# centreborelli/sat-bundleadjust

Measured on NVIDIA B200. Metric: lm_observation_iterations_per_s, higher is better.
Workload: dtype f64

## Files before the change

sat_bundleadjust_b200/csrc/sba_internal.cuh:

```cuda
#pragma once
#include <cuda_runtime.h>
#include <stdint.h>
#include <stdio.h>
#include <string>
#include <vector>

#include "../../include/sba_b200.h"
#include "sba_models.cuh"

namespace sba {

void set_error(const std::string& msg);

#define SBA_CUDA(expr)                                                                              \
    do {                                                                                            \
        cudaError_t _e = (expr);                                                                    \
        if (_e != cudaSuccess) {                                                                    \
            ::sba::set_error(std::string(#expr) + ": " + cudaGetErrorString(_e) + " (" + __FILE__ + ":" + \
                             std::to_string(__LINE__) + ")");                                       \
            return SBA_E_CUDA;                                                                      \
        }                                                                                           \
    } while (0)

#define SBA_TRY(expr)                \
// ... 73 lines not shown
    int *slice_block = nullptr, *slice_p0 = nullptr, *slice_p1 = nullptr;
    long long n_pairs = 0;
    int *tile_obs = nullptr;
    int n_tiles = 0;
    int n_schur_blocks = 0;

    double *x = nullptr, *x_new = nullptr, *g = nullptr, *sinv = nullptr, *delta = nullptr, *t1 = nullptr, *t2 = nullptr;
    double *camrec = nullptr, *camrec_new = nullptr;
    double *V = nullptr, *F = nullptr, *q = nullptr, *Z = nullptr;
    double *camsys_local = nullptr, *camsys = nullptr;
    double *S = nullptr;
    bool comm_split = false;
    int n_common = 0;
    double *cvec = nullptr;
    double *chol_work = nullptr;
    double *cam_partials = nullptr, *schur_partials = nullptr, *red_partials = nullptr;
    unsigned* counters = nullptr;
    double* scal = nullptr;
    double* h_scal = nullptr;
    double* r_out = nullptr;
    double* err_out = nullptr;
    double *io_x = nullptr;
    cudaEvent_t ev0 = nullptr, ev1 = nullptr;
    int launches = 0;
    std::vector<cudaEvent_t> ev_pool;
    int ev_used = 0;
    void* comm_buf = nullptr;
    void* comm_peer[16] = {nullptr};
    long long comm_cap = 0;
    unsigned long long comm_seq = 0;
    bool comm_ready = false;
    std::vector<void*> arena_chunks;
    std::vector<size_t> arena_chunk_bytes;
    char* arena_ptr = nullptr;
    size_t arena_left = 0;
    void* flush_buf = nullptr;
    size_t flush_bytes = 0;

    bool use_pcg = false;
    double pcg_tol = 1e-8;
    int pcg_max_it = 500;
    long long pcg_iterations = 0, pcg_solves = 0;
    double *pcg_vec = nullptr, *pcg_diag = nullptr, *pcg_L = nullptr, *pcg_w = nullptr, *pcg_s = nullptr;

    int engine = 0;
    int n_pts_fix_int = 0;
    std::vector<int> h_trk_new2old, h_obs_new2old;
    int *trk_new2old = nullptr, *obs_new2old = nullptr;
    void* pt_units[3] = {nullptr, nullptr, nullptr};
    int* pt_warp_unit0[3] = {nullptr, nullptr, nullptr};
    int pt_n_cta = 0;
    double *V2 = nullptr, *g2 = nullptr, *camsys2 = nullptr;
    long long* pt_cycles = nullptr;
    bool pt_obs_uploaded = false;
    bool pt_schur_mma = false;
    double *dsq = nullptr, *idsq = nullptr;
    double *dsqc = nullptr, *dsqc2 = nullptr, *idsqc = nullptr, *idsqc2 = nullptr;
    double *pt_partials = nullptr;
    double *osc = nullptr, *osc2 = nullptr;
    double *pt_records = nullptr;
    double *r_int = nullptr, *e_int = nullptr;
};
```

sat_bundleadjust_b200/csrc/sba_pattern.cuh:

```cuda
#pragma once
#include "sba_comm.cuh"
#include "sba_kernels.cuh"
#include "sba_pattern.h"

namespace sba {

constexpr int PT_CTAS = NUM_SMS;
constexpr int PT_THREADS = 512;
constexpr int PT_THREADS_LIGHT = 512;
constexpr int PT_THREADS_SCHUR = 384;
constexpr int PT_MAX_NS = 132;
constexpr int PT_RC = 3;

struct PatView {
    const PUnit* units;
    const int* warp_unit0;
    const double2* pts2d;
    const double* w;
    const double* cam_static;
    const double* rpc_tab;
    int M, P, n_cam_fix, n_cta;
    int debug_skip;
    long long* cycles;
};

__device__ __forceinline__ double step_value2(double x, double t, double d, double pa, double pb)
{
    return x + fma(pa, t, pb * d);
}

__device__ __forceinline__ bool invert_point_block_d2(double v0, double v1, double v2, double v3, double v4, double v5,
                                                      double d0, double d1, double d2, double reg, double G[6])
{
    const double a00 = v0 + reg * d0, a10 = v1, a20 = v2;
    const double a11 = v3 + reg * d1, a21 = v4, a22 = v5 + reg * d2;
    bool ok = a00 > 0.0;
    const double i00 = fast_rsqrt(a00);
    const double c10 = a10 * i00, c20 = a20 * i00;
    const double d11 = a11 - c10 * c10;
    ok = ok && d11 > 0.0;
    const double i11 = fast_rsqrt(d11);
    const double c21 = (a21 - c20 * c10) * i11;
    const double d22 = a22 - c20 * c20 - c21 * c21;
    ok = ok && d22 > 0.0;
    const double i22 = fast_rsqrt(d22);
    if (!ok) {
#pragma unroll
        for (int k = 0; k < 6; ++k) G[k] = 0.0;
        return false;
    }
    G[0] = i00; G[2] = i11; G[5] = i22;
    G[1] = -c10 * i00 * i11;
    G[4] = -c21 * i11 * i22;
    G[3] = -(c20 * i00 + c21 * G[1]) * i22;
    return true;
}

template <int NV>
__device__ __forceinline__ double cta_reduce_sum(double (&v)[NV], double* sm)
{
    warp_reduce_sum<NV>(v);
    const int lane = threadIdx.x & 31, warp = threadIdx.x >> 5, nw = blockDim.x >> 5;
    __syncthreads();
    if (lane == 0) {
#pragma unroll
        for (int k = 0; k < NV; ++k) sm[warp * NV + k] = v[k];
    }
    __syncthreads();
    double s = 0.0;
    if (threadIdx.x < NV)
        for (int wq = 0; wq < nw; ++wq) s += sm[wq * NV + threadIdx.x];
    __syncthreads();
    return s;
}

template <int NV>
__device__ __forceinline__ bool grid_sum_last(double block_total, double* partials, unsigned* counter, double* scal,
// ... 22 lines not shown
__device__ __forceinline__ void load_cameras_shared(const PatView& A, const double* __restrict__ camrec, double* s_cam,
                                                    double* s_rpc)
{
    for (int t = threadIdx.x; t < A.M * CAMREC_STRIDE; t += blockDim.x) s_cam[t] = camrec[t];
    if (MODEL == MODEL_RPC)
        for (int t = threadIdx.x; t < A.M * RPC_TAB_STRIDE; t += blockDim.x) s_rpc[t] = A.rpc_tab[t];
}

__device__ __forceinline__ int unit_camera(const PUnit& u, int k)
{
    const int nlo = __popc(u.mask_lo);
    return k < nlo ? (int)__fns(u.mask_lo, 0, k + 1) : 32 + (int)__fns(u.mask_hi, 0, k - nlo + 1);
}

struct LaneGeo {
    int L, T, k, t, cam;
    bool on;
};
__device__ __forceinline__ LaneGeo lane_geometry(const PUnit& u, int lane)
{
    LaneGeo g;
    g.L = u.L; g.T = min(32 / u.L, PT_MAX_T);
    g.t = lane / u.L; g.k = lane - g.t * u.L;
    g.on = g.t < g.T;
    g.cam = g.on ? unit_camera(u, g.k) : 0;
    return g;
}

__device__ __forceinline__ double slot_reduce(double v, const LaneGeo& g)
{
    for (int off = 1; off < g.T; off <<= 1) {
        const double o = __shfl_down_sync(0xffffffffu, v, (unsigned)(off * g.L) & 31);
        if (g.on && g.t + off < g.T) v += o;
    }
    return v;
}

template <int N>
__device__ __forceinline__ void slot_reduce_n(double (&v)[N], const LaneGeo& g)
{
    for (int off = 1; off < g.T; off <<= 1) {
        const unsigned delta = (unsigned)(off * g.L) & 31;
        const bool take = g.on && g.t + off < g.T;
        double o[N];
#pragma unroll
        for (int q = 0; q < N; ++q) o[q] = __shfl_down_sync(0xffffffffu, v[q], delta);
#pragma unroll
        for (int q = 0; q < N; ++q) if (take) v[q] += o[q];
    }
}

__device__ __forceinline__ void prefetch_l1(const void* p) { asm volatile("prefetch.global.L1 [%0];" ::"l"(p)); }

template <int MODEL, int NC>
__device__ __forceinline__ void eval_scaled(const double* __restrict__ rec, const double* __restrict__ rpc_j, double X, double Y,
                                            double Z, double2 sc, bool cam_free, bool pt_free, ObsEval<MODEL, NC>& e)
{
    double u, v;
    full_side<MODEL, NC, true>(rec, rpc_j, X, Y, Z, u, v, e.Jc, e.Jp);
    const double a0 = cam_free ? sc.x : 0.0, a1 = cam_free ? sc.y : 0.0;
#pragma unroll
    for (int k = 0; k < NC; ++k) { e.Jc[k] *= a0; e.Jc[NC + k] *= a1; }
    const double b0 = pt_free ? sc.x : 0.0, b1 = pt_free ? sc.y : 0.0;
#pragma unroll
    for (int k = 0; k < 3; ++k) { e.Jp[k] *= b0; e.Jp[3 + k] *= b1; }
}

template <int MODEL, int NC>
__global__ void __launch_bounds__(PT_THREADS, 1)
k_pt_assemble(PatView A, const double* __restrict__ x, const double* __restrict__ g, const double* __restrict__ idsq,
              const double* __restrict__ idsq_c, const double* __restrict__ delta, const double* __restrict__ scal,
              int initial, int ns, int loss, double f_scale, double* __restrict__ x_new, double* __restrict__ camrec_new,
              double* __restrict__ V_new, double* __restrict__ g_new, double2* __restrict__ osc_new, double* __restrict__ partials)
{
    constexpr int NU = NC * (NC + 1) / 2, NV = NU + NC;
    extern __shared__ double smem[];
    double* s_cam = smem;
    double* s_rpc = s_cam + A.M * CAMREC_STRIDE;
    double* s_acc = s_rpc + (MODEL == MODEL_RPC ? A.M * RPC_TAB_STRIDE : 0);
    const int lane = threadIdx.x & 31, warp = threadIdx.x >> 5, nw = blockDim.x >> 5;
    double* s_stage = s_acc + nw * A.M * NV;
    double* s_red = s_stage + nw * 9 * 33;
    const double pa = initial ? 0.0 : scal[SC_PA], pb = initial ? 0.0 : scal[SC_PB];
    if (threadIdx.x < A.M) {
        const int j = threadIdx.x;
        double v[MAX_CAM_PARAMS];
#pragma unroll
        for (int s = 0; s < MAX_CAM_PARAMS; ++s) {
            double val = 0.0;
            if (s < A.P) {
                if (s < NC) {
                    const size_t e = (size_t)j * NC + s;
                    const double xv = initial ? x[e] : step_value2(x[e], g[e] * idsq_c[e], delta[e], pa, pb);
                    if (blockIdx.x == 0) x_new[e] = xv;
                    val = j >= A.n_cam_fix ? xv : A.cam_static[(size_t)j * A.P + s];
                } else {
                    val = A.cam_static[(size_t)j * A.P + s];
                }
            }
            v[s] = val;
        }
        build_camrec(v, MODEL, s_cam + j * CAMREC_STRIDE);
    }
    if (MODEL == MODEL_RPC)
        for (int t = threadIdx.x; t < A.M * RPC_TAB_STRIDE; t += blockDim.x) s_rpc[t] = A.rpc_tab[t];
    for (int t = threadIdx.x; t < nw * A.M * NV; t += blockDim.x) s_acc[t] = 0.0;
    __syncthreads();
    if (blockIdx.x == 0)
        for (int t = threadIdx.x; t < A.M * CAMREC_STRIDE; t += blockDim.x) camrec_new[t] = s_cam[t];

    double cost[1] = {0.0};
    double* stg = s_stage + warp * 9 * 33;
    double* my_acc = s_acc + warp * A.M * NV;
    const int u0 = A.warp_unit0[blockIdx.x * nw + warp], u1 = A.debug_skip ? u0 : A.warp_unit0[blockIdx.x * nw + warp + 1];
    const long long cyc0 = clock64();
    for (int u = u0; u < u1; ++u) {
        const PUnit un = A.units[u];
        const LaneGeo G = lane_geometry(un, lane);
        const bool cam_free = G.cam >= A.n_cam_fix, pt_free = un.pts_free != 0;
        const double* rec = s_cam + G.cam * CAMREC_STRIDE;
        const double* rpc_j = MODEL == MODEL_RPC ? s_rpc + G.cam * RPC_TAB_STRIDE : nullptr;
        double acc[NV];
#pragma unroll
        for (int q = 0; q < NV; ++q) acc[q] = 0.0;
        for (int tb = 0; tb < un.ntrk; tb += G.T) {
            const int tt = tb + G.t;
            const bool on = G.on && tt < un.ntrk;
            const int nact = min(G.T, un.ntrk - tb);
// ... 58 lines not shown
            __syncwarp();
            for (int s = lane; s < 9 * nact; s += 32) {
                const int tr = s / 9, q = s - 9 * tr;
                const double* src = stg + q * 33 + tr * G.L;
                double tsum = 0.0;
                for (int m = 0; m < G.L; ++m) tsum += src[m];
                const int it = un.trk0 + tb + tr;
                if (q < 6) V_new[6 * (size_t)it + q] = tsum;
                else g_new[(size_t)ns + 3 * (size_t)it + (q - 6)] = tsum;
            }
            __syncwarp();
        }
        slot_reduce_n<NV>(acc, G);
        if (G.on && G.t == 0) {
            double* dst = my_acc + G.cam * NV;
#pragma unroll
            for (int q = 0; q < NV; ++q) dst[q] += acc[q];
        }
        __syncwarp();
    }
    if (A.cycles && lane == 0) A.cycles[blockIdx.x * nw + warp] = clock64() - cyc0;
    const double ctot = cta_reduce_sum<1>(cost, s_red);
    for (int t = threadIdx.x; t < A.M * NV; t += blockDim.x) {
        double sum = 0.0;
        for (int wq = 0; wq < nw; ++wq) sum += s_acc[wq * A.M * NV + t];
        partials[(size_t)t * A.n_cta + blockIdx.x] = sum;
    }
    if (threadIdx.x == 0) partials[(size_t)A.M * NV * A.n_cta + blockIdx.x] = ctot;
}

__device__ __forceinline__ void cam_scale_dev(const double* __restrict__ camsys, const double* __restrict__ dsq_c_cur,
                                              int first, int M, int NC, double* __restrict__ dsq_c_new,
                                              double* __restrict__ idsq_c_new, double* __restrict__ g_new, double* scal)
{
    const int ns = M * NC;
    for (int e = threadIdx.x; e < ns; e += blockDim.x) {
        const int j = e / NC, s = e - j * NC;
        const double diag = __ldcg(camsys + (size_t)j * NC * NC + s * NC + s);
        const double d = first ? (diag == 0.0 ? 1.0 : diag) : fmax(dsq_c_cur[e], diag);
        dsq_c_new[e] = d;
        idsq_c_new[e] = 1.0 / d;
        g_new[e] = __ldcg(camsys + (size_t)M * NC * NC + e);
    }
    if (threadIdx.x == 0) scal[SC_COST_NEW] = __ldcg(camsys + (size_t)M * NC * NC + ns);
}

template <int NC>
__global__ void __launch_bounds__(256)
k_pt_reduce_assemble(const double* __restrict__ partials, int n_cta, int M, double* __restrict__ camsys, int fold,
                     const double* __restrict__ dsq_c_cur, int first, double* __restrict__ dsq_c_new,
                     double* __restrict__ idsq_c_new, double* __restrict__ g_new, double* scal, unsigned* counter, CommFused comm)
{
    constexpr int NU = NC * (NC + 1) / 2, NV = NU + NC;
    const int lane = threadIdx.x & 31;
    const int total = M * NV + 1;
    const int v = blockIdx.x * (blockDim.x >> 5) + (threadIdx.x >> 5);
    if (v < total) {
        double s = 0.0;
        for (int b = lane; b < n_cta; b += 32) s += partials[(size_t)v * n_cta + b];
#pragma unroll
        for (int o = 16; o > 0; o >>= 1) s += __shfl_xor_sync(0xffffffffu, s, o);
        if (lane == 0) {
            if (v == M * NV) {
                camsys[(size_t)M * NC * NC + (size_t)M * NC] = s;
            } else {
                const int j = v / NV, q = v - j * NV;
                if (q < NU) {
                    int r = 0;
                    while ((r + 1) * (r + 2) / 2 <= q) ++r;
                    const int c = q - r * (r + 1) / 2;
                    camsys[(size_t)j * NC * NC + r * NC + c] = s;
                    camsys[(size_t)j * NC * NC + c * NC + r] = s;
                } else {
                    camsys[(size_t)M * NC * NC + (size_t)j * NC + (q - NU)] = s;
                }
            }
        }
    }
    if (!fold) return;
    __shared__ bool is_last;
    __threadfence();
    __syncthreads();
    if (threadIdx.x == 0) is_last = (atomicAdd(counter, 1u) == gridDim.x - 1);
    __syncthreads();
    if (!is_last) return;
    __threadfence();
    if (threadIdx.x == 0) *counter = 0u;
    if (comm.on) cta_allreduce(comm.c, camsys, M * NC * NC + M * NC + 1, comm.seq, scal);
    cam_scale_dev(camsys, dsq_c_cur, first, M, NC, dsq_c_new, idsq_c_new, g_new, scal);
}

__global__ void __launch_bounds__(256)
k_pt_cam_scale(const double* __restrict__ camsys, const double* __restrict__ dsq_c_cur, int first, int M, int NC,
               double* __restrict__ dsq_c_new, double* __restrict__ idsq_c_new, double* __restrict__ g_new, double* scal)
{
    cam_scale_dev(camsys, dsq_c_cur, first, M, NC, dsq_c_new, idsq_c_new, g_new, scal);
}

__device__ __forceinline__ void control_reg_dev(double* scal, double delta_arg, double reg_override)
{
    double Delta = delta_arg;
    if (Delta < 0.0) {
        Delta = sqrt(scal[SC_XS]);
        if (Delta == 0.0) Delta = 1.0;
    }
    scal[SC_DELTA] = Delta;
    if (reg_override >= 0.0) { scal[SC_REG] = reg_override; return; }
    const double gg = scal[SC_GG];
    const double qa = 0.5 * scal[SC_A], qb = -gg;
    const double to_tr = Delta / sqrt(gg);
    double ag = 0.0;
    ag = fmin(ag, to_tr * (qa * to_tr + qb));
    if (qa != 0.0) {
        const double ext = -0.5 * qb / qa;
        if (ext > 0.0 && ext < to_tr) ag = fmin(ag, ext * (qa * ext + qb));
    }
    scal[SC_REG] = -ag / (Delta * Delta);
}

__device__ __forceinline__ void control_tr2d_gram_dev(double* scal, double delta_arg)
{
    const double Delta = delta_arg < 0.0 ? scal[SC_DELTA] : delta_arg;
    const double gg = scal[SC_GG], gd = scal[SC_P_GD], dd = scal[SC_P_DD];
    const double b11 = scal[SC_A], c12 = scal[SC_P_C12], c22 = scal[SC_P_C22];
    const double t11 = scal[SC_P_T11], t1d = scal[SC_P_T1D], tdd = scal[SC_P_TDD];
    const double alpha = gg > 0.0 ? gd / gg : 0.0;
    double ww = dd - alpha * gd;
    if (!(ww > 1e-14 * dd)) ww = 0.0;
    const double b12 = c12 - alpha * b11, b22 = c22 - 2.0 * alpha * c12 + alpha * alpha * b11;
    const double t12 = t1d - alpha * t11, t22 = fmax(0.0, tdd - 2.0 * alpha * t1d + alpha * alpha * t11);
    const double n1 = sqrt(gg);
    const bool rank2 = ww > 0.0 && b22 > 0.0;
    const double n2 = rank2 ? sqrt(ww) : 1.0;
    const double B00 = b11 / (n1 * n1), B01 = rank2 ? b12 / (n1 * n2) : 0.0, B11 = rank2 ? b22 / (n2 * n2) : 1.0;
    const double gS0 = n1, gS1 = 0.0;
    double pS[2];
    solve_trust_region_2d(B00, B01, B11, gS0, gS1, Delta, pS);
    const double c1 = pS[0] / n1, c2 = rank2 ? pS[1] / n2 : 0.0;
    scal[SC_C1] = c1;
    scal[SC_C2] = c2;
    scal[SC_PA] = c1 - c2 * alpha;
    scal[SC_PB] = c2;
    scal[SC_PRED] = -(0.5 * (B00 * pS[0] * pS[0] + 2.0 * B01 * pS[0] * pS[1] + B11 * pS[1] * pS[1]) + gS0 * pS[0] + gS1 * pS[1]);
    scal[SC_STEPH] = sqrt(pS[0] * pS[0] + pS[1] * pS[1]);
    scal[SC_STEPN] = sqrt(fmax(0.0, c1 * c1 * t11 + 2.0 * c1 * c2 * t12 + c2 * c2 * t22));
    scal[SC_B22] = b22;
}

__global__ void k_pt_control_reg(double* scal, double delta_arg, double reg_override)
{
    if (threadIdx.x == 0 && blockIdx.x == 0) control_reg_dev(scal, delta_arg, reg_override);
}
__global__ void k_pt_control_tr2d(double* scal, double delta_arg)
{
    if (threadIdx.x == 0 && blockIdx.x == 0) control_tr2d_gram_dev(scal, delta_arg);
}

template <int MODEL, int NC>
__global__ void __launch_bounds__(PT_THREADS_LIGHT, 1)
k_pt_jvp1(PatView A, const double* __restrict__ x, const double* __restrict__ camrec, const double* __restrict__ V,
          const double* __restrict__ g, const double* __restrict__ dsq_c, const double* __restrict__ idsq_c,
          double* __restrict__ dsq, double* __restrict__ idsq, const double2* __restrict__ osc, int first, int ns,
          int count_cameras, int rank, double* partials, unsigned* counter, double* scal, int fold_ctl, double delta_arg, CommFused comm)
{
    extern __shared__ double smem[];
    double* s_cam = smem;
    double* s_rpc = s_cam + A.M * CAMREC_STRIDE;
    double* s_t1c = s_rpc + (MODEL == MODEL_RPC ? A.M * RPC_TAB_STRIDE : 0);
    double* s_red = s_t1c + ns;
    const int lane = threadIdx.x & 31, warp = threadIdx.x >> 5, nw = blockDim.x >> 5;
    load_cameras_shared<MODEL>(A, camrec, s_cam, s_rpc);
    for (int e = threadIdx.x; e < ns; e += blockDim.x) s_t1c[e] = g[e] * idsq_c[e];
    __syncthreads();
    double acc[4] = {0.0, 0.0, 0.0, 0.0};
    double gmax = 0.0;
    if (blockIdx.x == 0 && count_cameras) {
        for (int e = threadIdx.x; e < ns; e += blockDim.x) {
            const double gv = g[e], xv = x[e];
            acc[0] += gv * gv * idsq_c[e];
            acc[1] += xv * xv * dsq_c[e];
            acc[2] += xv * xv;
            gmax = fmax(gmax, fabs(gv));
        }
    }
    const int u0 = A.warp_unit0[blockIdx.x * nw + warp], u1 = A.debug_skip ? u0 : A.warp_unit0[blockIdx.x * nw + warp + 1];
    const long long cyc0 = clock64();
    for (int u = u0; u < u1; ++u) {
        const PUnit un = A.units[u];
        const LaneGeo G = lane_geometry(un, lane);
        const bool cam_free = G.cam >= A.n_cam_fix, pt_free = un.pts_free != 0;
        const double* rec = s_cam + G.cam * CAMREC_STRIDE;
        const double* rpc_j = MODEL == MODEL_RPC ? s_rpc + G.cam * RPC_TAB_STRIDE : nullptr;
        const double* t1c = s_t1c + G.cam * NC;
        for (int tb = 0; tb < un.ntrk; tb += G.T) {
            const int tt = tb + G.t;
            if (!(G.on && tt < un.ntrk)) continue;
            if (tt + G.T < un.ntrk) {
                const size_t in = (size_t)(un.trk0 + tt + G.T), en = (size_t)ns + 3 * in;
                prefetch_l1(osc + (size_t)un.obs0 + (size_t)(tt + G.T) * G.L + G.k);
                prefetch_l1(x + en); prefetch_l1(g + en); prefetch_l1(dsq + en); prefetch_l1(V + 6 * in);
            }
            const int i = un.trk0 + tt;
            const size_t a = (size_t)un.obs0 + (size_t)tt * G.L + G.k;
            const size_t e3 = (size_t)ns + 3 * (size_t)i;
            const double2 sc = osc[a];
            const double X = x[e3], Y = x[e3 + 1], Z = x[e3 + 2];
            const double vd[3] = {V[6 * (size_t)i], V[6 * (size_t)i + 3], V[6 * (size_t)i + 5]};
            double t1p[3], d2[3], gp[3];
#pragma unroll
            for (int q = 0; q < 3; ++q) {
                gp[q] = g[e3 + q];
                d2[q] = first ? (vd[q] == 0.0 ? 1.0 : vd[q]) : fmax(dsq[e3 + q], vd[q]);
                const double id = fast_rcp(d2[q]);
                t1p[q] = gp[q] * id;
                if (G.k == 0) { dsq[e3 + q] = d2[q]; idsq[e3 + q] = id; }
            }
            if (G.k == 0) {
                acc[0] += gp[0] * t1p[0] + gp[1] * t1p[1] + gp[2] * t1p[2];
                acc[1] += X * X * d2[0] + Y * Y * d2[1] + Z * Z * d2[2];
                acc[2] += X * X + Y * Y + Z * Z;
                gmax = fmax(gmax, fmax(fabs(gp[0]), fmax(fabs(gp[1]), fabs(gp[2]))));
            }
            ObsEval<MODEL, NC> e;
// ... 15 lines not shown
    __shared__ int slots[4];
    if (threadIdx.x == 0) { slots[0] = SC_GG; slots[1] = SC_XS; slots[2] = SC_XX; slots[3] = SC_A; }
    __syncthreads();
    const bool last = grid_sum_last<4>(tot, partials, counter, scal, slots);
    if (last && comm.on) cta_allreduce(comm.c, scal + SC_COST, SC_GGN - SC_COST, comm.seq, scal);
    if (last && fold_ctl && threadIdx.x == 0) control_reg_dev(scal, delta_arg, -1.0);
}

__host__ __device__ inline int pt_block_offset(int j, int jp, int M, int NC)
{
    return NC * NC * (j * M - j * (j - 1) / 2 + (jp - j));
}

template <int NC>
struct SchurTasks {
    static constexpr int NCH = (NC + PT_RC - 1) / PT_RC;
    int ntask, npass, npar, par;
    int ka[2], kb[2], hh[2];
    bool tv[2];
    __device__ __forceinline__ void unit(int L, int lane)
    {
        ntask = L * (L + 1) / 2 * NCH;
        npass = (ntask + 63) / 64;
        npar = ntask <= 16 ? 32 / ntask : 1;
        par = npar > 1 ? lane / ntask : 0;
    }
    __device__ __forceinline__ void pass(int L, int lane, int p)
    {
#pragma unroll
        for (int q = 0; q < 2; ++q) {
            int tau = p * 64 + q * 32 + lane;
            tv[q] = tau < ntask;
            if (npar > 1) { tau = lane - par * ntask; tv[q] = q == 0 && par < npar; }
            const int pr = tv[q] ? tau / NCH : 0;
            hh[q] = tv[q] ? tau - pr * NCH : 0;
            int a = 0, rem = pr;
            while (rem >= L - a) { rem -= L - a; ++a; }
            ka[q] = a; kb[q] = a + rem;
        }
    }
};

template <int NC> __host__ __device__ constexpr int pt_record_doubles() { return (2 * PT_RC * NC + NC) * 32; }

template <int MODEL, int NC>
__global__ void __launch_bounds__(PT_THREADS_SCHUR, 1)
k_pt_schur(PatView A, const double* __restrict__ x, const double* __restrict__ camrec, const double* __restrict__ V,
           const double* __restrict__ g, const double* __restrict__ dsq, const double2* __restrict__ osc,
           const double* __restrict__ scal, int ns, double* __restrict__ records, double* __restrict__ partials, double* bad_points)
{
    constexpr int ZS = NC * 3, ZP = ZS + 1;
    constexpr int NA = PT_RC * NC;
    constexpr int REC = pt_record_doubles<NC>();
    extern __shared__ double smem[];
    const int nS = NC * NC * (A.M * (A.M + 1) / 2);
    double* s_cam = smem;
    double* s_rpc = s_cam + A.M * CAMREC_STRIDE;
    double* s_Z = s_rpc + (MODEL == MODEL_RPC ? A.M * RPC_TAB_STRIDE : 0);
    const int lane = threadIdx.x & 31, warp = threadIdx.x >> 5, nw = blockDim.x >> 5;
    const double reg = scal[SC_REG];
    load_cameras_shared<MODEL>(A, camrec, s_cam, s_rpc);
    __syncthreads();
    double* zs = s_Z + (size_t)warp * (32 * ZP + PT_RC * 3);
    int nbad = 0;
    const int u0 = A.warp_unit0[blockIdx.x * nw + warp], u1 = A.debug_skip ? u0 : A.warp_unit0[blockIdx.x * nw + warp + 1];
    SchurTasks<NC> tk;
    const long long cyc0 = clock64();
    for (int u = u0; u < u1; ++u) {
        const PUnit un = A.units[u];
        const LaneGeo G = lane_geometry(un, lane);
        const bool cam_free = G.cam >= A.n_cam_fix, pt_free = un.pts_free != 0;
        const double* rec = s_cam + G.cam * CAMREC_STRIDE;
        const double* rpc_j = MODEL == MODEL_RPC ? s_rpc + G.cam * RPC_TAB_STRIDE : nullptr;
        tk.unit(G.L, lane);
        for (int pass = 0; pass < tk.npass; ++pass) {
            tk.pass(G.L, lane, pass);
            double acc[2][NA], accR[NC];
#pragma unroll
            for (int q = 0; q < 2; ++q)
#pragma unroll
                for (int m = 0; m < NA; ++m) acc[q][m] = 0.0;
#pragma unroll
            for (int r = 0; r < NC; ++r) accR[r] = 0.0;
            for (int tb = 0; tb < un.ntrk; tb += G.T) {
                const int tt = tb + G.t;
                const bool on = G.on && tt < un.ntrk;
                const int nact = min(G.T, un.ntrk - tb);
                if (G.on && tt + G.T < un.ntrk) {
                    const size_t in = (size_t)(un.trk0 + tt + G.T), en = (size_t)ns + 3 * in;
                    prefetch_l1(osc + (size_t)un.obs0 + (size_t)(tt + G.T) * G.L + G.k);
                    prefetch_l1(x + en); prefetch_l1(g + en); prefetch_l1(dsq + en); prefetch_l1(V + 6 * in);
                }
                if (on) {
                    const int i = un.trk0 + tt;
                    const size_t a = (size_t)un.obs0 + (size_t)tt * G.L + G.k;
                    const size_t e3 = (size_t)ns + 3 * (size_t)i;
                    const double2 sc = osc[a];
                    const double X = x[e3], Y = x[e3 + 1], Z = x[e3 + 2];
                    const double* v = V + 6 * (size_t)i;
                    double Gm[6], qv[3] = {0.0, 0.0, 0.0};
                    bool ok = false;
                    if (pt_free) ok = invert_point_block_d2(v[0], v[1], v[2], v[3], v[4], v[5], dsq[e3], dsq[e3 + 1], dsq[e3 + 2], reg, Gm);
                    if (!ok) {
#pragma unroll
                        for (int m = 0; m < 6; ++m) Gm[m] = 0.0;
                        if (pt_free && G.k == 0 && pass == 0) ++nbad;
                    } else {
                        const double g0 = g[e3], g1 = g[e3 + 1], g2 = g[e3 + 2];
                        qv[0] = Gm[0] * g0;
                        qv[1] = Gm[1] * g0 + Gm[2] * g1;
                        qv[2] = Gm[3] * g0 + Gm[4] * g1 + Gm[5] * g2;
                    }
                    ObsEval<MODEL, NC> e;
                    eval_scaled<MODEL, NC>(rec, rpc_j, X, Y, Z, sc, cam_free, pt_free, e);
                    double* z = zs + lane * ZP;
#pragma unroll
                    for (int r = 0; r < NC; ++r) {
                        const double w0 = e.Jc[r] * e.Jp[0] + e.Jc[NC + r] * e.Jp[3];
// ... 2 lines not shown
                        const double z0 = w0 * Gm[0], z1 = w0 * Gm[1] + w1 * Gm[2], z2 = w0 * Gm[3] + w1 * Gm[4] + w2 * Gm[5];
                        z[3 * r] = z0; z[3 * r + 1] = z1; z[3 * r + 2] = z2;
                        if (pass == 0) accR[r] = fma(z2, qv[2], fma(z1, qv[1], fma(z0, qv[0], accR[r])));
                    }
                }
                __syncwarp();
                for (int ts = tk.par; ts < nact; ts += tk.npar) {
#pragma unroll
                    for (int q = 0; q < 2; ++q) {
                        if (!tk.tv[q]) continue;
                        const double* za = zs + (ts * G.L + tk.ka[q]) * ZP + tk.hh[q] * PT_RC * 3;
                        const double* zb = zs + (ts * G.L + tk.kb[q]) * ZP;
                        double Ar[PT_RC * 3];
#pragma unroll
                        for (int m = 0; m < PT_RC * 3; ++m) Ar[m] = za[m];
#pragma unroll
                        for (int s = 0; s < NC; ++s) {
                            const double b0 = zb[3 * s], b1 = zb[3 * s + 1], b2 = zb[3 * s + 2];
#pragma unroll
                            for (int r = 0; r < PT_RC; ++r)
                                acc[q][r * NC + s] = fma(Ar[3 * r + 2], b2, fma(Ar[3 * r + 1], b1, fma(Ar[3 * r], b0, acc[q][r * NC + s])));
                        }
                    }
                }
                __syncwarp();
            }
            if (tk.npar > 1) {
                for (int off = 1; off < tk.npar; off <<= 1) {
#pragma unroll
                    for (int m = 0; m < NA; ++m) {
                        const double o = __shfl_down_sync(0xffffffffu, acc[0][m], (unsigned)(off * tk.ntask));
                        if (tk.tv[0] && tk.par + off < tk.npar) acc[0][m] += o;
                    }
                }
            }
            double* rp = records + (size_t)(un.rec + pass) * REC;
#pragma unroll
            for (int q = 0; q < 2; ++q) {
                if (pass * 64 + q * 32 >= tk.ntask) continue;
#pragma unroll
                for (int m = 0; m < NA; ++m) zs[lane * NA + m] = acc[q][m];
                __syncwarp();
                for (int e = lane; e < 32 * NA; e += 32) rp[q * 32 * NA + e] = zs[e];
                __syncwarp();
            }
            if (pass == 0) {
                slot_reduce_n<NC>(accR, G);
#pragma unroll
                for (int r = 0; r < NC; ++r) rp[(2 * NA + r) * 32 + lane] = accR[r];
            }
        }
    }
    if (A.cycles && lane == 0) A.cycles[blockIdx.x * nw + warp] = clock64() - cyc0;
    if (nbad) atomicAdd(bad_points, (double)nbad);
    __threadfence();
    __syncthreads();
    {
        constexpr int NCH = SchurTasks<NC>::NCH;
        constexpr int MU = 4;
        const int cu0 = A.warp_unit0[blockIdx.x * nw], cu1 = A.warp_unit0[(blockIdx.x + 1) * nw];
        const int ncu = cu1 - cu0;
        int* s_units = reinterpret_cast<int*>(s_Z);
        const int cap = (int)(((size_t)nw * (32 * ZP + PT_RC * 3) * sizeof(double)) / (4 * sizeof(int))) - 1;
        for (int c0 = 0; c0 < max(ncu, 1); c0 += cap) {
            const int nc_here = min(cap, ncu - c0);
            __syncthreads();
            for (int q = threadIdx.x; q < nc_here; q += blockDim.x) {
                const PUnit un = A.units[cu0 + c0 + q];
                s_units[4 * q] = (int)un.mask_lo; s_units[4 * q + 1] = (int)un.mask_hi; s_units[4 * q + 2] = un.L; s_units[4 * q + 3] = un.rec;
            }
            if (threadIdx.x == 0) { s_units[4 * nc_here] = 0; }
            __syncthreads();
            const int nrow = (A.M * (A.M + 1) / 2) * NC;
            for (int task = threadIdx.x; task < nrow + A.M; task += blockDim.x) {
                double sum[NC];
                const bool is_S = task < nrow;
                int ja = 0, jb = 0, h = 0, mrow = 0;
                size_t t0;
                if (is_S) {
                    int bq = task / NC;
                    const int r = task - bq * NC;
                    t0 = (size_t)bq * NC * NC + (size_t)r * NC;
                    while (bq >= A.M - ja) { bq -= A.M - ja; ++ja; }
                    jb = ja + bq;
                    h = r / PT_RC; mrow = (r - h * PT_RC) * NC;
                } else {
                    ja = jb = task - nrow;
                    t0 = (size_t)nS + (size_t)ja * NC;
                }
#pragma unroll
                for (int c = 0; c < NC; ++c) sum[c] = c0 == 0 ? 0.0 : partials[(t0 + c) * A.n_cta + blockIdx.x];
                for (int q0 = 0; q0 < nc_here; q0 += MU) {
                    double val[MU][NC];
#pragma unroll
                    for (int qq = 0; qq < MU; ++qq) {
                        const int q = min(q0 + qq, nc_here - 1);
                        const unsigned long long mask = ((unsigned long long)(unsigned)s_units[4 * q + 1] << 32) | (unsigned)s_units[4 * q];
                        const int L = s_units[4 * q + 2], rec0 = s_units[4 * q + 3];
                        const bool has = q0 + qq < nc_here && ((mask >> ja) & 1ull) && ((mask >> jb) & 1ull);
                        const int ka = __popcll(mask & ((1ull << ja) - 1ull)), kb = __popcll(mask & ((1ull << jb) - 1ull));
                        const double* src;
                        int stride;
                        if (is_S) {
                            const int tau = (ka * L - ka * (ka - 1) / 2 + (kb - ka)) * NCH + h;
                            src = records + (size_t)(rec0 + (tau >> 6)) * REC + (((tau >> 5) & 1) * 32 + (tau & 31)) * NA + mrow;
                            stride = 1;
                        } else {
                            src = records + (size_t)rec0 * REC + (2 * NA) * 32 + ka;
                            stride = 32;
                        }
#pragma unroll
                        for (int c = 0; c < NC; ++c) val[qq][c] = has ? __ldcg(src + c * stride) : 0.0;
                    }
#pragma unroll
                    for (int qq = 0; qq < MU; ++qq)
#pragma unroll
                        for (int c = 0; c < NC; ++c) sum[c] += val[qq][c];
                }
#pragma unroll
                for (int c = 0; c < NC; ++c) partials[(t0 + c) * A.n_cta + blockIdx.x] = sum[c];
            }
        }
    }
}

__device__ __forceinline__ void mma_f64_884(double (&d)[2], double a, double b)
{
    asm volatile("mma.sync.aligned.m8n8k4.row.col.f64.f64.f64.f64 {%0, %1}, {%2}, {%3}, {%0, %1};" : "+d"(d[0]), "+d"(d[1]) : "d"(a), "d"(b));
}
template <int NC> __host__ __device__ constexpr int pt_record_doubles_mma() { return PT_MMA_TILES * 64 + NC * 32; }

template <int MODEL, int NC>
__global__ void __launch_bounds__(PT_THREADS_SCHUR, 1)
k_pt_schur_mma(PatView A, const double* __restrict__ x, const double* __restrict__ camrec, const double* __restrict__ V,
           const double* __restrict__ g, const double* __restrict__ dsq, const double2* __restrict__ osc,
           const double* __restrict__ scal, int ns, double* __restrict__ records, double* __restrict__ partials, double* bad_points)
{
    constexpr int ZS = NC * 3, ZP = ZS + 1;
    constexpr int NTP = PT_MMA_TILES;
    constexpr int REC = pt_record_doubles_mma<NC>();
    extern __shared__ double smem[];
    const int nS = NC * NC * (A.M * (A.M + 1) / 2);
    double* s_cam = smem;
    double* s_rpc = s_cam + A.M * CAMREC_STRIDE;
    double* s_Z = s_rpc + (MODEL == MODEL_RPC ? A.M * RPC_TAB_STRIDE : 0);
    const int lane = threadIdx.x & 31, warp = threadIdx.x >> 5, nw = blockDim.x >> 5;
    const double reg = scal[SC_REG];
    load_cameras_shared<MODEL>(A, camrec, s_cam, s_rpc);
    __syncthreads();
    double* zs = s_Z + (size_t)warp * (32 * ZP + PT_RC * 3);
    int nbad = 0;
    const int u0 = A.warp_unit0[blockIdx.x * nw + warp], u1 = A.debug_skip ? u0 : A.warp_unit0[blockIdx.x * nw + warp + 1];
    const int frow = lane >> 2, fk = lane & 3;
    const long long cyc0 = clock64();
    for (int u = u0; u < u1; ++u) {
        const PUnit un = A.units[u];
        const LaneGeo G = lane_geometry(un, lane);
        const bool cam_free = G.cam >= A.n_cam_fix, pt_free = un.pts_free != 0;
        const double* rec = s_cam + G.cam * CAMREC_STRIDE;
        const double* rpc_j = MODEL == MODEL_RPC ? s_rpc + G.cam * RPC_TAB_STRIDE : nullptr;
        const int nrows = G.L * NC, R = (nrows + 7) >> 3, ntile = R * (R + 1) / 2, npass = (ntile + NTP - 1) / NTP;
        int foff[6];
        bool fok[6];
#pragma unroll
        for (int i = 0; i < 6; ++i) {
            const int row = 8 * i + frow, pos = row / NC;
            fok[i] = row < nrows && fk < 3;
            foff[i] = fok[i] ? pos * ZP + (row - pos * NC) * 3 + fk : 0;
        }
        for (int pass = 0; pass < npass; ++pass) {
            double C[NTP][2], accR[NC];
#pragma unroll
            for (int q = 0; q < NTP; ++q) { C[q][0] = 0.0; C[q][1] = 0.0; }
#pragma unroll
            for (int r = 0; r < NC; ++r) accR[r] = 0.0;
            for (int tb = 0; tb < un.ntrk; tb += G.T) {
                const int tt = tb + G.t;
                const bool on = G.on && tt < un.ntrk;
                const int nact = min(G.T, un.ntrk - tb);
                if (G.on && tt + G.T < un.ntrk) {
                    const size_t in = (size_t)(un.trk0 + tt + G.T), en = (size_t)ns + 3 * in;
                    prefetch_l1(osc + (size_t)un.obs0 + (size_t)(tt + G.T) * G.L + G.k);
                    prefetch_l1(x + en); prefetch_l1(g + en); prefetch_l1(dsq + en); prefetch_l1(V + 6 * in);
                }
                if (on) {
                    const int i = un.trk0 + tt;
                    const size_t a = (size_t)un.obs0 + (size_t)tt * G.L + G.k;
                    const size_t e3 = (size_t)ns + 3 * (size_t)i;
                    const double2 sc = osc[a];
                    const double X = x[e3], Y = x[e3 + 1], Z = x[e3 + 2];
                    const double* v = V + 6 * (size_t)i;
                    double Gm[6], qv[3] = {0.0, 0.0, 0.0};
                    bool ok = false;
                    if (pt_free) ok = invert_point_block_d2(v[0], v[1], v[2], v[3], v[4], v[5], dsq[e3], dsq[e3 + 1], dsq[e3 + 2], reg, Gm);
                    if (!ok) {
#pragma unroll
                        for (int m = 0; m < 6; ++m) Gm[m] = 0.0;
                        if (pt_free && G.k == 0 && pass == 0) ++nbad;
                    } else {
                        const double g0 = g[e3], g1 = g[e3 + 1], g2 = g[e3 + 2];
                        qv[0] = Gm[0] * g0;
                        qv[1] = Gm[1] * g0 + Gm[2] * g1;
// ... 108 lines not shown
                        if (is_S) {
                            const int grow = ka * NC + r_in;
#pragma unroll
                            for (int c = 0; c < NC; ++c) {
                                const int gcol = kb * NC + c;
                                const int lo = min(grow, gcol), hi = max(grow, gcol);
                                const int ti = lo >> 3, tj = hi >> 3, tile = tj * (tj + 1) / 2 + ti, ps = tile / NTP;
                                const double* src = records + (size_t)(rec0 + ps) * REC + (tile - ps * NTP) * 64 + (lo & 7) * 8 + (hi & 7);
                                val[qq][c] = has ? __ldcg(src) : 0.0;
                            }
                        } else {
                            const double* src = records + (size_t)rec0 * REC + (size_t)NTP * 64 + ka;
#pragma unroll
                            for (int c = 0; c < NC; ++c) val[qq][c] = has ? __ldcg(src + c * 32) : 0.0;
                        }
                    }
#pragma unroll
                    for (int qq = 0; qq < MU; ++qq)
#pragma unroll
                        for (int c = 0; c < NC; ++c) sum[c] += val[qq][c];
                }
#pragma unroll
                for (int c = 0; c < NC; ++c) partials[(t0 + c) * A.n_cta + blockIdx.x] = sum[c];
            }
        }
    }
}

template <int NC>
__device__ __forceinline__ void reduce_schur_store(int v, double val, int M, double* __restrict__ S)
{
    const int ns = M * NC, nS = NC * NC * (M * (M + 1) / 2);
    if (v >= nS) { S[(size_t)ns * ns + (v - nS)] = val; return; }
    int b = v / (NC * NC);
    const int rs = v - b * NC * NC, r = rs / NC, c = rs - r * NC;
    int j = 0;
    while (b >= M - j) { b -= M - j; ++j; }
    const int jp = j + b;
    S[(size_t)(j * NC + r) + (size_t)(jp * NC + c) * ns] = val;
    if (j != jp) S[(size_t)(jp * NC + c) + (size_t)(j * NC + r) * ns] = val;
}

template <int NC>
__global__ void __launch_bounds__(512)
k_pt_reduce_schur(const double* __restrict__ partials, int n_cta, int M, int n_cam_fix, const double* __restrict__ camsys,
                  const double* __restrict__ dsq_c, double* scal, int add_diag, double* __restrict__ S, CommFused comm,
                  unsigned* counter)
{
    const int lane = threadIdx.x & 31;
    const int ns = M * NC, nS = NC * NC * (M * (M + 1) / 2), total = nS + ns;
    const int gw = blockIdx.x * (blockDim.x >> 5) + (threadIdx.x >> 5), nwarps = gridDim.x * (blockDim.x >> 5);
    const int parity = (int)(comm.seq & 1ull);
    double* mine = comm.on ? comm.c.data[comm.c.me] + (long long)parity * comm.c.cap : nullptr;
    const double reg = scal[SC_REG];
    for (int v = gw; v < total; v += nwarps) {
        double s = 0.0;
        for (int b = lane; b < n_cta; b += 32) s += partials[(size_t)v * n_cta + b];
#pragma unroll
        for (int o = 16; o > 0; o >>= 1) s += __shfl_xor_sync(0xffffffffu, s, o);
        if (lane != 0) continue;
        double val;
        if (v >= nS) {
            val = (add_diag ? -camsys[(size_t)M * NC * NC + (v - nS)] : 0.0) + s;
        } else {
            int b = v / (NC * NC);
            const int rs = v - b * NC * NC, r = rs / NC, c = rs - r * NC;
            int j = 0;
            while (b >= M - j) { b -= M - j; ++j; }
            val = -s;
            if (b == 0 && add_diag) {
                val += camsys[(size_t)j * NC * NC + r * NC + c];
                if (r == c) val += (j < n_cam_fix) ? 1.0 : reg * dsq_c[(size_t)j * NC + r];
            }
        }
        if (comm.on) mine[v] = val;
        else reduce_schur_store<NC>(v, val, M, S);
    }
    if (!comm.on) return;
    __threadfence_system();
    __shared__ bool last;
    __shared__ int ok;
    __syncthreads();
    if (threadIdx.x == 0) { last = (atomicAdd(counter, 1u) == gridDim.x - 1); ok = 1; }
    __syncthreads();
    const CommView& c = comm.c;
    if (last) {
        __threadfence_system();
        if (threadIdx.x < c.world && threadIdx.x != c.me)
            st_release_sys(c.flag[threadIdx.x] + parity * COMM_MAX_RANKS + c.me, comm.seq);
        if (threadIdx.x == 0) *counter = 0u;
    }
    if (threadIdx.x < c.world && threadIdx.x != c.me) {
        const unsigned long long* f = c.flag[c.me] + parity * COMM_MAX_RANKS + threadIdx.x;
        const long long t0 = clock64();
        while (ld_acquire_sys(f) < comm.seq) {
            if (clock64() - t0 > c.timeout_cycles) { ok = 0; break; }
        }
    }
    __syncthreads();
    if (!ok) {
        if (threadIdx.x == 0) scal[SC_COMM_FAIL] = 1.0;
        return;
    }
    for (int v = gw; v < total; v += nwarps) {
        double part = 0.0;
        if (lane < c.world) part = ld_volatile_f64(c.data[lane] + (long long)parity * c.cap + v);
// ... 169 lines not shown
```

Measured before the change: 2.807 billion.

## Add programmatic dependent launch overlap and per-stage timing probes to pattern kernels

Adds griddepcontrol trigger/wait calls to the pattern kernels so a dependent kernel can start its prologue (camera loads into shared memory, L1 prefetch of the first unit's data) while the previous kernel finishes. It also moves the resetting of bad-point and Cholesky-failure counters into the control step, and adds optional per-stage clock and globaltimer instrumentation. The overlap only takes effect if the host launches with the PDL attribute, which is not visible here. The timing hooks insert extra syncs and fences only when the stages buffer is set.

```diff
diff --git a/sat_bundleadjust_b200/csrc/sba_internal.cuh b/sat_bundleadjust_b200/csrc/sba_internal.cuh
--- a/sat_bundleadjust_b200/csrc/sba_internal.cuh
+++ b/sat_bundleadjust_b200/csrc/sba_internal.cuh
@@ -149,6 +149,7 @@
     int pt_n_cta = 0;
     double *V2 = nullptr, *g2 = nullptr, *camsys2 = nullptr;
     long long* pt_cycles = nullptr;
+    long long* pt_stages = nullptr;
     bool pt_obs_uploaded = false;
     bool pt_schur_mma = false;
     double *dsq = nullptr, *idsq = nullptr;
diff --git a/sat_bundleadjust_b200/csrc/sba_pattern.cuh b/sat_bundleadjust_b200/csrc/sba_pattern.cuh
--- a/sat_bundleadjust_b200/csrc/sba_pattern.cuh
+++ b/sat_bundleadjust_b200/csrc/sba_pattern.cuh
@@ -22,7 +22,18 @@
     int M, P, n_cam_fix, n_cta;
     int debug_skip;
     long long* cycles;
+    long long* stages;
 };
+
+constexpr int PT_STAGE_SLOTS = 32;
+__device__ __forceinline__ long long global_ns()
+{
+    unsigned long long t;
+    asm volatile("mov.u64 %0, %%globaltimer;" : "=l"(t));
+    return (long long)t;
+}
+#define PT_STAGE(slot, value) \
+    do { if (A.stages && threadIdx.x == 0) A.stages[(size_t)blockIdx.x * PT_STAGE_SLOTS + (slot)] = (value); } while (0)
 
 __device__ __forceinline__ double step_value2(double x, double t, double d, double pa, double pb)
 {
@@ -151,6 +162,9 @@
 
 __device__ __forceinline__ void prefetch_l1(const void* p) { asm volatile("prefetch.global.L1 [%0];" ::"l"(p)); }
 
+__device__ __forceinline__ void pdl_wait() { asm volatile("griddepcontrol.wait;" ::: "memory"); }
+__device__ __forceinline__ void pdl_trigger() { asm volatile("griddepcontrol.launch_dependents;" ::: "memory"); }
+
 template <int MODEL, int NC>
 __device__ __forceinline__ void eval_scaled(const double* __restrict__ rec, const double* __restrict__ rpc_j, double X, double Y,
                                             double Z, double2 sc, bool cam_free, bool pt_free, ObsEval<MODEL, NC>& e)
@@ -173,6 +187,7 @@
               double* __restrict__ V_new, double* __restrict__ g_new, double2* __restrict__ osc_new, double* __restrict__ partials)
 {
     constexpr int NU = NC * (NC + 1) / 2, NV = NU + NC;
+    pdl_trigger();
     extern __shared__ double smem[];
     double* s_cam = smem;
     double* s_rpc = s_cam + A.M * CAMREC_STRIDE;
@@ -337,6 +352,7 @@
                      double* __restrict__ idsq_c_new, double* __restrict__ g_new, double* scal, unsigned* counter, CommFused comm)
 {
     constexpr int NU = NC * (NC + 1) / 2, NV = NU + NC;
+    pdl_wait();
     const int lane = threadIdx.x & 31;
     const int total = M * NV + 1;
     const int v = blockIdx.x * (blockDim.x >> 5) + (threadIdx.x >> 5);
@@ -384,6 +400,8 @@
 
 __device__ __forceinline__ void control_reg_dev(double* scal, double delta_arg, double reg_override)
 {
+    scal[SC_BAD_POINTS] = 0.0;
+    scal[SC_CHOL_FAIL] = 0.0;
     double Delta = delta_arg;
     if (Delta < 0.0) {
         Delta = sqrt(scal[SC_XS]);
@@ -454,6 +472,7 @@
     double* s_t1c = s_rpc + (MODEL == MODEL_RPC ? A.M * RPC_TAB_STRIDE : 0);
     double* s_red = s_t1c + ns;
     const int lane = threadIdx.x & 31, warp = threadIdx.x >> 5, nw = blockDim.x >> 5;
+    pdl_trigger();
     load_cameras_shared<MODEL>(A, camrec, s_cam, s_rpc);
     for (int e = threadIdx.x; e < ns; e += blockDim.x) s_t1c[e] = g[e] * idsq_c[e];
     __syncthreads();
@@ -575,18 +594,33 @@
     constexpr int ZS = NC * 3, ZP = ZS + 1;
     constexpr int NA = PT_RC * NC;
     constexpr int REC = pt_record_doubles<NC>();
+    PT_STAGE(0, clock64());
+    PT_STAGE(5, global_ns());
     extern __shared__ double smem[];
     const int nS = NC * NC * (A.M * (A.M + 1) / 2);
     double* s_cam = smem;
     double* s_rpc = s_cam + A.M * CAMREC_STRIDE;
     double* s_Z = s_rpc + (MODEL == MODEL_RPC ? A.M * RPC_TAB_STRIDE : 0);
     const int lane = threadIdx.x & 31, warp = threadIdx.x >> 5, nw = blockDim.x >> 5;
+    pdl_trigger();
+    load_cameras_shared<MODEL>(A, camrec, s_cam, s_rpc);
+    const int u0 = A.warp_unit0[blockIdx.x * nw + warp], u1 = A.debug_skip ? u0 : A.warp_unit0[blockIdx.x * nw + warp + 1];
+    if (u0 < u1) {
+        const PUnit un = A.units[u0];
+        const LaneGeo G = lane_geometry(un, lane);
+        if (G.on && G.t < un.ntrk) {
+            const size_t in = (size_t)(un.trk0 + G.t);
+            prefetch_l1(osc + (size_t)un.obs0 + (size_t)G.t * G.L + G.k);
+            prefetch_l1(x + (size_t)ns + 3 * in); prefetch_l1(g + (size_t)ns + 3 * in); prefetch_l1(V + 6 * in);
+        }
+    }
+    __syncthreads();
+    PT_STAGE(7, clock64());
+    pdl_wait();
+    PT_STAGE(1, clock64());
     const double reg = scal[SC_REG];
-    load_cameras_shared<MODEL>(A, camrec, s_cam, s_rpc);
-    __syncthreads();
     double* zs = s_Z + (size_t)warp * (32 * ZP + PT_RC * 3);
     int nbad = 0;
-    const int u0 = A.warp_unit0[blockIdx.x * nw + warp], u1 = A.debug_skip ? u0 : A.warp_unit0[blockIdx.x * nw + warp + 1];
     SchurTasks<NC> tk;
     const long long cyc0 = clock64();
     for (int u = u0; u < u1; ++u) {
@@ -695,9 +729,12 @@
         }
     }
     if (A.cycles && lane == 0) A.cycles[blockIdx.x * nw + warp] = clock64() - cyc0;
+    if (A.stages && lane == 0) A.stages[(size_t)blockIdx.x * PT_STAGE_SLOTS + 8 + warp] = clock64();
     if (nbad) atomicAdd(bad_points, (double)nbad);
     __threadfence();
     __syncthreads();
+    PT_STAGE(2, clock64());
+    long long clk_store = 0;
     {
         constexpr int NCH = SchurTasks<NC>::NCH;
         constexpr int MU = 4;
@@ -715,55 +752,69 @@
             if (threadIdx.x == 0) { s_units[4 * nc_here] = 0; }
             __syncthreads();
             const int nrow = (A.M * (A.M + 1) / 2) * NC;
-            for (int task = threadIdx.x; task < nrow + A.M; task += blockDim.x) {
+            for (int tbase = 0; tbase < nrow + A.M; tbase += blockDim.x) {
+                const int task = tbase + threadIdx.x;
                 double sum[NC];
-                const bool is_S = task < nrow;
-                int ja = 0, jb = 0, h = 0, mrow = 0;
-                size_t t0;
-                if (is_S) {
-                    int bq = task / NC;
-                    const int r = task - bq * NC;
-                    t0 = (size_t)bq * NC * NC + (size_t)r * NC;
-                    while (bq >= A.M - ja) { bq -= A.M - ja; ++ja; }
-                    jb = ja + bq;
-                    h = r / PT_RC; mrow = (r - h * PT_RC) * NC;
-                } else {
-                    ja = jb = task - nrow;
-                    t0 = (size_t)nS + (size_t)ja * NC;
-                }
-#pragma unroll
-                for (int c = 0; c < NC; ++c) sum[c] = c0 == 0 ? 0.0 : partials[(t0 + c) * A.n_cta + blockIdx.x];
-                for (int q0 = 0; q0 < nc_here; q0 += MU) {
-                    double val[MU][NC];
-#pragma unroll
-                    for (int qq = 0; qq < MU; ++qq) {
-                        const int q = min(q0 + qq, nc_here - 1);
-                        const unsigned long long mask = ((unsigned long long)(unsigned)s_units[4 * q + 1] << 32) | (unsigned)s_units[4 * q];
-                        const int L = s_units[4 * q + 2], rec0 = s_units[4 * q + 3];
-                        const bool has = q0 + qq < nc_here && ((mask >> ja) & 1ull) && ((mask >> jb) & 1ull);
-                        const int ka = __popcll(mask & ((1ull << ja) - 1ull)), kb = __popcll(mask & ((1ull << jb) - 1ull));
-                        const double* src;
-                        int stride;
-                        if (is_S) {
-                            const int tau = (ka * L - ka * (ka - 1) / 2 + (kb - ka)) * NCH + h;
-                            src = records + (size_t)(rec0 + (tau >> 6)) * REC + (((tau >> 5) & 1) * 32 + (tau & 31)) * NA + mrow;
-                            stride = 1;
-                        } else {
-                            src = records + (size_t)rec0 * REC + (2 * NA) * 32 + ka;
-                            stride = 32;
+                size_t t0 = 0;
+                if (task < nrow + A.M) {
+                    const bool is_S = task < nrow;
+                    int ja = 0, jb = 0, h = 0, mrow = 0;
+                    if (is_S) {
+                        int bq = task / NC;
+                        const int r = task - bq * NC;
+                        t0 = (size_t)bq * NC * NC + (size_t)r * NC;
+                        while (bq >= A.M - ja) { bq -= A.M - ja; ++ja; }
+                        jb = ja + bq;
+                        h = r / PT_RC; mrow = (r - h * PT_RC) * NC;
+                    } else {
+                        ja = jb = task - nrow;
+                        t0 = (size_t)nS + (size_t)ja * NC;
+                    }
+#pragma unroll
+                    for (int c = 0; c < NC; ++c) sum[c] = c0 == 0 ? 0.0 : partials[(t0 + c) * A.n_cta + blockIdx.x];
+                    for (int q0 = 0; q0 < nc_here; q0 += MU) {
+                        double val[MU][NC];
+#pragma unroll
+                        for (int qq = 0; qq < MU; ++qq) {
+                            const int q = min(q0 + qq, nc_here - 1);
+                            const unsigned long long mask = ((unsigned long long)(unsigned)s_units[4 * q + 1] << 32) | (unsigned)s_units[4 * q];
+                            const int L = s_units[4 * q + 2], rec0 = s_units[4 * q + 3];
+                            const bool has = q0 + qq < nc_here && ((mask >> ja) & 1ull) && ((mask >> jb) & 1ull);
+                            const int ka = __popcll(mask & ((1ull << ja) - 1ull)), kb = __popcll(mask & ((1ull << jb) - 1ull));
+                            const double* src;
+                            int stride;
+                            if (is_S) {
+                                const int tau = (ka * L - ka * (ka - 1) / 2 + (kb - ka)) * NCH + h;
+                                src = records + (size_t)(rec0 + (tau >> 6)) * REC + (((tau >> 5) & 1) * 32 + (tau & 31)) * NA + mrow;
+                                stride = 1;
+                            } else {
+                                src = records + (size_t)rec0 * REC + (2 * NA) * 32 + ka;
+                                stride = 32;
+                            }
+#pragma unroll
+                            for (int c = 0; c < NC; ++c) val[qq][c] = has ? __ldcg(src + c * stride) : 0.0;
                         }
 #pragma unroll
-                        for (int c = 0; c < NC; ++c) val[qq][c] = has ? __ldcg(src + c * stride) : 0.0;
+                        for (int qq = 0; qq < MU; ++qq)
+#pragma unroll
+                            for (int c = 0; c < NC; ++c) sum[c] += val[qq][c];
                     }
-#pragma unroll
-                    for (int qq = 0; qq < MU; ++qq)
-#pragma unroll
-                        for (int c = 0; c < NC; ++c) sum[c] += val[qq][c];
-                }
-#pragma unroll
-                for (int c = 0; c < NC; ++c) partials[(t0 + c) * A.n_cta + blockIdx.x] = sum[c];
-            }
-        }
+                }
+                long long tm1 = 0;
+                if (A.stages) { __syncthreads(); tm1 = clock64(); }
+                if (task < nrow + A.M) {
+#pragma unroll
+                    for (int c = 0; c < NC; ++c) partials[(t0 + c) * A.n_cta + blockIdx.x] = sum[c];
+                }
+                if (A.stages) { __threadfence(); __syncthreads(); clk_store += clock64() - tm1; }
+            }
+        }
+    }
+    if (A.stages) {
+        const long long t4 = clock64();
+        PT_STAGE(3, t4 - clk_store);
+        PT_STAGE(4, t4);
+        PT_STAGE(6, global_ns());
     }
 }
 
@@ -788,9 +839,11 @@
     double* s_rpc = s_cam + A.M * CAMREC_STRIDE;
     double* s_Z = s_rpc + (MODEL == MODEL_RPC ? A.M * RPC_TAB_STRIDE : 0);
     const int lane = threadIdx.x & 31, warp = threadIdx.x >> 5, nw = blockDim.x >> 5;
+    pdl_trigger();
+    load_cameras_shared<MODEL>(A, camrec, s_cam, s_rpc);
+    __syncthreads();
+    pdl_wait();
     const double reg = scal[SC_REG];
-    load_cameras_shared<MODEL>(A, camrec, s_cam, s_rpc);
-    __syncthreads();
     double* zs = s_Z + (size_t)warp * (32 * ZP + PT_RC * 3);
     int nbad = 0;
     const int u0 = A.warp_unit0[blockIdx.x * nw + warp], u1 = A.debug_skip ? u0 : A.warp_unit0[blockIdx.x * nw + warp + 1];
@@ -1005,6 +1058,7 @@
     const int gw = blockIdx.x * (blockDim.x >> 5) + (threadIdx.x >> 5), nwarps = gridDim.x * (blockDim.x >> 5);
     const int parity = (int)(comm.seq & 1ull);
     double* mine = comm.on ? comm.c.data[comm.c.me] + (long long)parity * comm.c.cap : nullptr;
+    pdl_wait();
     const double reg = scal[SC_REG];
     for (int v = gw; v < total; v += nwarps) {
         double s = 0.0;
```

Result: faster. 2.839 billion (median of 6 runs) (+1.1%).
